# cloneofsimo/lora

Hardware: AMD Instinct MI355X
Metric: train steps/sec SD1.5 rank-4 512^2 (train_lora_dreambooth.py step) (higher is better)
Workload: dtype bf16

## Files before the change

include/lora_amd.h:

```cpp
#ifndef LORA_AMD_H
#define LORA_AMD_H

#include <stddef.h>
#include <stdint.h>

#ifdef __cplusplus
extern "C" {
#endif

#define LORA_AMD_ABI_VERSION 7

#define LORA_AMD_OK 0
#define LORA_AMD_EINVAL (-1)
#define LORA_AMD_ERANK (-2)
#define LORA_AMD_ELAUNCH (-3)
#define LORA_AMD_EWORKSPACE (-4)
#define LORA_AMD_EUNSUPPORTED (-5)

#define LORA_AMD_MAX_RANK 64

#define LORA_AMD_F32 0
#define LORA_AMD_F16 1
#define LORA_AMD_BF16 2

// ... 445 lines not shown
                                  int32_t r, int32_t act_dtype, float scale, float dropout_p, uint64_t seed, uint64_t offset,
                                  const uint64_t *offset_dev, void *stream);
int lora_amd_sum_parts(const float *part, int32_t nparts, int64_t stride, float *out, int64_t n, void *stream);


size_t lora_amd_sumsq_workspace(int64_t n);
int lora_amd_sumsq(const float *g, int64_t n, float *out_sumsq, void *workspace,
                   size_t workspace_bytes, void *stream);

typedef struct lora_amd_adamw_group {
  int64_t begin, end;
  float lr;
  float weight_decay;
} lora_amd_adamw_group;

int lora_amd_clip_adamw(float *p, float *g, float *exp_avg, float *exp_avg_sq,
                        int64_t n, const lora_amd_adamw_group *groups_dev,
                        int32_t n_groups, const float *sumsq, float grad_scale,
                        float max_norm, float beta1, float beta2, float eps,
                        int64_t step, int32_t zero_grad, void *stream);

int lora_amd_clip_adamw_dev(float *p, float *g, float *exp_avg, float *exp_avg_sq,
                            int64_t n, const lora_amd_adamw_group *groups_dev,
                            int32_t n_groups, const float *sumsq, float grad_scale,
                            float max_norm, float beta1, float beta2, float eps,
                            const int64_t *step_dev, const float *scaler, int32_t zero_grad, void *stream);
int lora_amd_step_advance(int64_t *step_dev, void *stream);

int lora_amd_loss_scale_update(float *state, const float *sumsq, int64_t *step_dev, float growth_factor,
                               float backoff_factor, int32_t growth_interval, void *stream);

int lora_amd_ti_rows_step(void *table, const void *table_grad, const int64_t *ids_dev, int32_t n_tokens,
                          int32_t hidden, int32_t table_dtype, float *rows, float *exp_avg, float *exp_avg_sq,
                          float lr, float beta1, float beta2, float eps, float weight_decay, float grad_scale,
                          int64_t step, float decay_lambda, float target_norm, void *stream);


size_t lora_amd_groupnorm_workspace(int32_t B, int32_t C, int32_t HW, int32_t groups);
int lora_amd_groupnorm_supported(int32_t B, int32_t C, int32_t HW, int32_t groups);
int lora_amd_groupnorm_fwd(const void *x, const void *gamma, const void *beta, void *y, float *stats,
                           void *workspace, size_t workspace_bytes, int32_t B, int32_t C, int32_t HW,
                           int32_t groups, float eps, int32_t act, int32_t dtype, void *stream);
int lora_amd_groupnorm_bwd(const void *x, const void *gout, const void *gamma, const void *beta,
                           const float *stats, void *dx, void *workspace, size_t workspace_bytes, int32_t B,
                           int32_t C, int32_t HW, int32_t groups, int32_t act, int32_t dtype, void *stream);

size_t lora_amd_groupnorm_nhwc_workspace(int32_t B, int32_t C, int32_t HW, int32_t groups);
int lora_amd_groupnorm_nhwc_fwd(const void *x, const void *gamma, const void *beta, const float *addend, void *y,
                                float *aff, void *workspace, size_t workspace_bytes, int32_t B, int32_t C, int32_t HW,
                                int32_t groups, float eps, int32_t act, int32_t dtype, void *stream);
int lora_amd_groupnorm_nhwc_bwd(const void *x, const void *gout, const void *gamma, const float *aff, void *dx,
                                void *workspace, size_t workspace_bytes, int32_t B, int32_t C, int32_t HW,
                                int32_t groups, int32_t act, int32_t dtype, void *stream);

int lora_amd_layernorm_supported(int32_t K);
int lora_amd_layernorm_fwd(const void *x, const void *gamma, const void *beta, void *y, float *stats, int64_t M,
                           int32_t K, float eps, int32_t dtype, void *stream);
int lora_amd_layernorm_bwd(const void *x, const void *gout, const void *gamma, const float *stats, void *dx,
                           int64_t M, int32_t K, int32_t dtype, void *stream);
int lora_amd_add_layernorm_fwd(const void *x, const void *res, const void *gamma, const void *beta, void *sum_out,
                               void *y, float *stats, int64_t M, int32_t K, float eps, int32_t dtype, void *stream);
int lora_amd_add_layernorm_bwd(const void *x, const void *gout, const void *gsum, const void *gamma,
                               const float *stats, void *dx, int64_t M, int32_t K, int32_t dtype, void *stream);

int lora_amd_geglu_fwd(const void *y, int64_t ldy, void *out, int64_t ldo, int64_t M, int32_t inner, int32_t dtype,
                       void *stream);
int lora_amd_geglu_bwd(const void *y, int64_t ldy, const void *gout, int64_t ldg, void *gy, int64_t ldgy, int64_t M,
                       int32_t inner, int32_t dtype, void *stream);

#ifdef __cplusplus
}
#endif
#endif
```

lora_amd/_C.py:

```python
from __future__ import annotations

import ctypes as C
import os
from typing import Dict, Optional, Sequence, Tuple

import torch

_HERE = os.path.dirname(os.path.abspath(__file__))
LIB_PATH = os.path.join(_HERE, "csrc", "liblora_amd.so")

OK = 0
F32, F16, BF16 = 0, 1, 2
FACTOR_RK, FACTOR_KR = 0, 1
ROUND_REFERENCE, ROUND_ONCE, ROUND_DITHER = 0, 1, 2
MAX_RANK = 64
ABI_VERSION = 7

_DT = {torch.float32: F32, torch.float16: F16, torch.bfloat16: BF16}

SYMBOLS = (
    "lora_amd_abi_version", "lora_amd_last_error", "lora_amd_target_arch",
    "lora_amd_merge_plan", "lora_amd_merge_batched", "lora_amd_merge_set_tuning", "lora_amd_merge_step_set_tuning", "lora_amd_rank16_mfma", "lora_amd_factors_mfma_set_tuning",
    "lora_amd_merge_step_plan", "lora_amd_merge_step",
    "lora_amd_rowdot", "lora_amd_rowdot_masked", "lora_amd_rank_update",
    "lora_amd_colreduce_workspace", "lora_amd_colreduce",
    "lora_amd_rowdot_batched", "lora_amd_colreduce_batched", "lora_amd_chol_inverse_batched",
    "lora_amd_ragged_plan", "lora_amd_rowdot_ragged", "lora_amd_colreduce_ragged", "lora_amd_sub_ragged",
    "lora_amd_rowdot16_planes_plan", "lora_amd_rowdot16_planes", "lora_amd_rowdot16_planes_packed", "lora_amd_thin_pack",
    "lora_amd_split16_ragged", "lora_amd_split16_transpose",
    "lora_amd_split16_residual", "lora_amd_thin_gram", "lora_amd_thin_apply", "lora_amd_thin_rotate", "lora_amd_thin_select", "lora_amd_thin_clamp",
    "lora_amd_linear_plan", "lora_amd_linear_fwd", "lora_amd_linear_bwd_g", "lora_amd_linear_bwd_x",
    "lora_amd_linear_bwd_factors", "lora_amd_linear_bwd_factors_drop", "lora_amd_linear_bwd_factors_heads",
    "lora_amd_linear_factors_self_plan", "lora_amd_linear_factors_self_plan_rows", "lora_amd_linear_bwd_factors_self",
    "lora_amd_linear_factors_self_ragged_plan", "lora_amd_linear_bwd_factors_self_ragged",
    "lora_amd_factors_mfma_plan", "lora_amd_factor_pack_plan", "lora_amd_factor_pack",
    "lora_amd_factors_mfma_ragged_plan", "lora_amd_linear_bwd_factors_mfma_ragged", "lora_amd_factors_mfma_block_map",
    "lora_amd_linear_bwd_factors_mfma_ragged_mapped",
    "lora_amd_linear_gemm_fwd_heads",
    "lora_amd_reduce_batched", "lora_amd_linear_gemm_supported", "lora_amd_linear_gemm_fwd",
    "lora_amd_ws_config", "lora_amd_ws_packed_elems", "lora_amd_ws_pack", "lora_amd_linear_ws", "lora_amd_linear_ws_heads",
    "lora_amd_conv_plan", "lora_amd_conv_down_fwd", "lora_amd_conv_up_fwd", "lora_amd_conv_bwd_g", "lora_amd_conv_bwd_x",
    "lora_amd_conv3_nhwc_plan", "lora_amd_conv3_nhwc_pack", "lora_amd_conv3_nhwc_down_fwd", "lora_amd_conv3_nhwc_bwd_dx",
    "lora_amd_conv3_nhwc_bwd_down", "lora_amd_sum_parts",
    "lora_amd_conv3_nhwc_pack_plan", "lora_amd_conv3_nhwc_pack_batched", "lora_amd_conv3_nhwc_fwd_fused",
    "lora_amd_linear_bwd_g_blocks", "lora_amd_linear_bwd_g_folded",
    "lora_amd_sumsq_workspace", "lora_amd_sumsq", "lora_amd_clip_adamw", "lora_amd_clip_adamw_dev",
    "lora_amd_step_advance", "lora_amd_loss_scale_update", "lora_amd_ti_rows_step",
    "lora_amd_groupnorm_workspace", "lora_amd_groupnorm_supported", "lora_amd_groupnorm_fwd", "lora_amd_groupnorm_bwd",
    "lora_amd_geglu_fwd", "lora_amd_geglu_bwd",
    "lora_amd_layernorm_supported", "lora_amd_layernorm_fwd", "lora_amd_layernorm_bwd",
    "lora_amd_groupnorm_nhwc_workspace", "lora_amd_groupnorm_nhwc_fwd", "lora_amd_groupnorm_nhwc_bwd",
    "lora_amd_add_layernorm_fwd", "lora_amd_add_layernorm_bwd",
    "lora_amd_linear_gemm_fwd_rowscale", "lora_amd_rank_update_rowscale", "lora_amd_conv_up_fwd_rowscale",
)


class HipExtensionMissing(RuntimeError):
    pass


class FactorsSelfPlan(C.Structure):
    _fields_ = [("supported", C.c_int32), ("rank_tile", C.c_int32), ("nparts", C.c_int32), ("reserved", C.c_int32),
                ("up_part_floats", C.c_int64), ("down_part_floats", C.c_int64)]


class SelfSite(C.Structure):
    _fields_ = [
        ("g", C.c_void_p), ("x", C.c_void_p), ("down", C.c_void_p), ("up", C.c_void_p),
        ("up_part", C.c_void_p), ("down_part", C.c_void_p),
        ("ldg", C.c_int64), ("ldx", C.c_int64), ("M", C.c_int64),
        ("N", C.c_int32), ("K", C.c_int32), ("r", C.c_int32), ("scale", C.c_float),
        ("g_head_dim", C.c_int32), ("g_head_pad", C.c_int32), ("x_head_dim", C.c_int32), ("x_head_pad", C.c_int32),
        ("rows_per_block", C.c_int32), ("nsplit", C.c_int32), ("kt_g", C.c_int32), ("logL_g", C.c_int32),
        ("kt_x", C.c_int32), ("logL_x", C.c_int32), ("tile_g", C.c_int32), ("nct_g", C.c_int32),
        ("tile_x", C.c_int32), ("nct_x", C.c_int32),
        ("reserved0", C.c_int32), ("reserved", C.c_int32),
        ("block_begin", C.c_int64),
    ]


class FactorsMfmaPlan(C.Structure):
    _fields_ = [("supported", C.c_int32), ("lds_class", C.c_int32), ("rank_tile", C.c_int32),
                ("rows_per_block", C.c_int32), ("nparts", C.c_int32), ("lds_bytes", C.c_int32),
                ("blocks_per_wg", C.c_int32), ("reserved", C.c_int32),
                ("up_part_floats", C.c_int64), ("down_part_floats", C.c_int64),
                ("pack_up_elems", C.c_int64), ("pack_down_elems", C.c_int64)]


class PackSite(C.Structure):
    _fields_ = [("down", C.c_void_p), ("up", C.c_void_p), ("pk_down", C.c_void_p), ("pk_up", C.c_void_p),
                ("N", C.c_int32), ("K", C.c_int32), ("r", C.c_int32), ("reserved", C.c_int32), ("begin", C.c_int64)]


class FmSite(C.Structure):
    _fields_ = [
        ("g", C.c_void_p), ("x", C.c_void_p), ("pk_up", C.c_void_p), ("pk_down", C.c_void_p),
        ("up_part", C.c_void_p), ("down_part", C.c_void_p),
        ("ldg", C.c_int64), ("ldx", C.c_int64), ("M", C.c_int64),
        ("N", C.c_int32), ("K", C.c_int32), ("r", C.c_int32), ("scale", C.c_float),
        ("g_head_dim", C.c_int32), ("g_head_pad", C.c_int32), ("x_head_dim", C.c_int32), ("x_head_pad", C.c_int32),
        ("rows_per_block", C.c_int32), ("blocks_per_wg", C.c_int32),
        ("resident_is_x", C.c_int32), ("cw", C.c_int32), ("nchunk", C.c_int32), ("x_head_magic", C.c_int32),
        ("g_head_magic", C.c_int32), ("lds_bytes", C.c_int32),
        ("block_begin", C.c_int64),
# ... 236 lines not shown
    lib.lora_amd_linear_gemm_supported.restype = lib.lora_amd_linear_gemm_fwd.restype = C.c_int
    lib.lora_amd_linear_gemm_fwd_rowscale.argtypes = [vp, i64, vp, i64, vp, vp, i64, vp, vp, vp, i64, i32, i32, i32, i32,
                                                      f32, vp, i32, i64, i32, vp]
    lib.lora_amd_rank_update_rowscale.argtypes = [vp, i64, vp, vp, i64, i32, i32, i32, i32, i32, f32, vp, i32, i64, f32,
                                                  u64, u64, vp]
    lib.lora_amd_conv_up_fwd_rowscale.argtypes = [vp, vp, vp, i32, i32, i32, i32, i32, i32, i32, f32, vp, i32, i64, f32,
                                                  u64, u64, vp]
    for name in ("lora_amd_linear_gemm_fwd_rowscale", "lora_amd_rank_update_rowscale", "lora_amd_conv_up_fwd_rowscale"):
        getattr(lib, name).restype = C.c_int
    lib.lora_amd_ws_config.argtypes = [i32, C.POINTER(i32), C.POINTER(i32)]
    lib.lora_amd_ws_packed_elems.argtypes = [i32, i32]
    lib.lora_amd_ws_packed_elems.restype = i64
    lib.lora_amd_ws_pack.argtypes = [vp, i64, i64, i32, i32, i32, vp, vp]
    lib.lora_amd_linear_ws.argtypes = [vp, i64, i64, i32, i32, C.POINTER(WsSite), i32, i32, vp]
    lib.lora_amd_linear_ws_heads.argtypes = [vp, i64, i64, i32, i32, i32, i32, C.POINTER(WsSite), i32, i32, vp]
    lib.lora_amd_ws_config.restype = lib.lora_amd_ws_pack.restype = lib.lora_amd_linear_ws.restype = C.c_int
    lib.lora_amd_linear_ws_heads.restype = C.c_int
    lib.lora_amd_conv_plan.argtypes = [i32, i32, i32, i32, i32, i32, i32, C.POINTER(ConvPlan)]
    lib.lora_amd_conv_down_fwd.argtypes = [vp, vp, vp, vp, vp, i32, i32, i32, i32, i32, i32, i32, i32, vp]
    lib.lora_amd_conv_up_fwd.argtypes = [vp, vp, vp, i32, i32, i32, i32, i32, i32, i32, f32, f32, u64, u64, vp, vp]
    lib.lora_amd_conv_bwd_g.argtypes = [vp, vp, vp, vp, vp, vp, vp, i32, i32, i32, i32, i32, i32, i32, f32, f32, u64,
                                        u64, vp, vp]
    lib.lora_amd_conv_bwd_x.argtypes = [vp, vp, vp, vp, vp, i32, i32, i32, i32, i32, i32, i32, i32, vp]
    lib.lora_amd_conv3_nhwc_plan.argtypes = [i32, i32, i32, i32, i32, C.POINTER(Conv3NhwcPlan)]
    lib.lora_amd_conv3_nhwc_pack.argtypes = [vp, i32, i32, i32, vp, vp, vp]
    lib.lora_amd_conv3_nhwc_down_fwd.argtypes = [vp, vp, vp, vp, i32, i32, i32, i32, i32, i32, vp]
    lib.lora_amd_conv3_nhwc_bwd_dx.argtypes = [vp, vp, vp, i32, i32, i32, i32, i32, i32, vp]
    lib.lora_amd_conv3_nhwc_bwd_down.argtypes = [vp, vp, vp, i32, i32, i32, i32, i32, i32, vp]
    lib.lora_amd_sum_parts.argtypes = [vp, i32, i64, vp, i64, vp]
    lib.lora_amd_conv3_nhwc_pack_plan.argtypes = [C.POINTER(Conv3PackSite), i32, C.POINTER(i64)]
    lib.lora_amd_conv3_nhwc_pack_batched.argtypes = [vp, i32, i64, i32, vp]
    lib.lora_amd_conv3_nhwc_fwd_fused.argtypes = [vp, vp, vp, vp, vp, vp, vp, i32, i32, i32, i32, i32, i32, i32, f32, f32,
                                                  u64, u64, vp, vp]
    lib.lora_amd_linear_bwd_g_blocks.argtypes = [i64, i32, i32, C.POINTER(i64)]
    lib.lora_amd_linear_bwd_g_folded.argtypes = [vp, i64, vp, vp, vp, vp, vp, vp, i64, i32, i32, i32, i32, f32, f32, u64,
                                                 u64, vp, vp]
    for name in ("lora_amd_conv3_nhwc_plan", "lora_amd_conv3_nhwc_pack", "lora_amd_conv3_nhwc_down_fwd",
                 "lora_amd_conv3_nhwc_bwd_dx", "lora_amd_conv3_nhwc_bwd_down", "lora_amd_sum_parts",
                 "lora_amd_conv3_nhwc_pack_plan", "lora_amd_conv3_nhwc_pack_batched", "lora_amd_conv3_nhwc_fwd_fused",
                 "lora_amd_linear_bwd_g_blocks", "lora_amd_linear_bwd_g_folded"):
        getattr(lib, name).restype = C.c_int
    lib.lora_amd_groupnorm_workspace.argtypes = [i32, i32, i32, i32]
    lib.lora_amd_groupnorm_workspace.restype = sz
    lib.lora_amd_groupnorm_supported.argtypes = [i32, i32, i32, i32]
    lib.lora_amd_groupnorm_fwd.argtypes = [vp, vp, vp, vp, vp, vp, sz, i32, i32, i32, i32, f32, i32, i32, vp]
    lib.lora_amd_groupnorm_bwd.argtypes = [vp, vp, vp, vp, vp, vp, vp, sz, i32, i32, i32, i32, i32, i32, vp]
    lib.lora_amd_geglu_fwd.argtypes = [vp, i64, vp, i64, i64, i32, i32, vp]
    lib.lora_amd_geglu_bwd.argtypes = [vp, i64, vp, i64, vp, i64, i64, i32, i32, vp]
    lib.lora_amd_groupnorm_nhwc_workspace.argtypes = [i32, i32, i32, i32]
    lib.lora_amd_groupnorm_nhwc_workspace.restype = sz
    lib.lora_amd_groupnorm_nhwc_fwd.argtypes = [vp, vp, vp, vp, vp, vp, vp, sz, i32, i32, i32, i32, f32, i32, i32, vp]
    lib.lora_amd_groupnorm_nhwc_bwd.argtypes = [vp, vp, vp, vp, vp, vp, sz, i32, i32, i32, i32, i32, i32, vp]
    lib.lora_amd_groupnorm_nhwc_fwd.restype = lib.lora_amd_groupnorm_nhwc_bwd.restype = C.c_int
    lib.lora_amd_add_layernorm_fwd.argtypes = [vp, vp, vp, vp, vp, vp, vp, i64, i32, f32, i32, vp]
    lib.lora_amd_add_layernorm_bwd.argtypes = [vp, vp, vp, vp, vp, vp, i64, i32, i32, vp]
    lib.lora_amd_add_layernorm_fwd.restype = lib.lora_amd_add_layernorm_bwd.restype = C.c_int
    lib.lora_amd_layernorm_supported.argtypes = [i32]
    lib.lora_amd_layernorm_fwd.argtypes = [vp, vp, vp, vp, vp, i64, i32, f32, i32, vp]
    lib.lora_amd_layernorm_bwd.argtypes = [vp, vp, vp, vp, vp, i64, i32, i32, vp]
    for name in ("lora_amd_groupnorm_supported", "lora_amd_groupnorm_fwd", "lora_amd_groupnorm_bwd",
                 "lora_amd_geglu_fwd", "lora_amd_geglu_bwd", "lora_amd_layernorm_supported",
                 "lora_amd_layernorm_fwd", "lora_amd_layernorm_bwd"):
        getattr(lib, name).restype = C.c_int
    for name in ("lora_amd_conv_plan", "lora_amd_conv_down_fwd", "lora_amd_conv_up_fwd", "lora_amd_conv_bwd_g",
                 "lora_amd_conv_bwd_x"):
        getattr(lib, name).restype = C.c_int
    for name in ("lora_amd_linear_plan", "lora_amd_linear_fwd", "lora_amd_linear_bwd_g", "lora_amd_linear_bwd_x",
                 "lora_amd_reduce_batched"):
        getattr(lib, name).restype = C.c_int
    for name in ("lora_amd_merge_plan", "lora_amd_merge_batched", "lora_amd_merge_set_tuning", "lora_amd_rowdot",
                 "lora_amd_rowdot_masked", "lora_amd_rank_update", "lora_amd_colreduce", "lora_amd_sumsq",
                 "lora_amd_clip_adamw"):
        getattr(lib, name).restype = C.c_int


def load() -> Optional[C.CDLL]:
    global _lib, _load_error
    if _lib is not None or _load_error is not None:
        return _lib
    if not os.path.exists(LIB_PATH):
        _load_error = f"{LIB_PATH} not built (run `python -c 'import __graft_entry__ as g; g.build()'`)"
        return None
    try:
        lib = C.CDLL(LIB_PATH)
        _declare(lib)
        if lib.lora_amd_abi_version() != ABI_VERSION:
            raise OSError(f"ABI version {lib.lora_amd_abi_version()} != {ABI_VERSION} (rebuild: make -C lora_amd/csrc)")
        _lib = lib
    except OSError as e:
        _load_error = f"cannot load {LIB_PATH}: {e}"
    return _lib


def available() -> bool:
    return load() is not None


def require() -> C.CDLL:
    lib = load()
    if lib is None:
        raise HipExtensionMissing(
            "lora_amd: the HIP extension is required for device tensors and is not loadable: " + str(_load_error))
    return lib


def _check(rc: int, what: str) -> None:
# ... 1534 lines not shown
    gy = torch.empty(y.shape, dtype=y.dtype, device=y.device)
    _check(require().lora_amd_geglu_bwd(y2.data_ptr(), y2.stride(0), g2.data_ptr(), g2.stride(0), gy.data_ptr(),
                                        2 * inner, y2.shape[0], inner, dtype_code(y.dtype), _stream()),
           "lora_amd_geglu_bwd")
    return gy


def layernorm_supported(K: int) -> bool:
    return bool(require().lora_amd_layernorm_supported(K))


def layernorm_fwd(x: torch.Tensor, gamma: torch.Tensor, beta: torch.Tensor, eps: float, *,
                  out: Optional[torch.Tensor] = None, stats: Optional[torch.Tensor] = None) -> Tuple[torch.Tensor, torch.Tensor]:
    _dev_check(x, gamma, beta, out, stats)
    K = x.shape[-1]
    M = x.numel() // K
    if out is None:
        y = torch.empty_like(x)
    elif out.dtype != x.dtype or out.shape != x.shape or not out.is_contiguous():
        raise ValueError("layernorm_fwd: out must be a contiguous tensor of x's shape and dtype")
    else:
        y = out
    if stats is None:
        stats = torch.empty(M, 2, dtype=torch.float32, device=x.device)
    elif stats.dtype != torch.float32 or tuple(stats.shape) != (M, 2) or not stats.is_contiguous():
        raise ValueError(f"layernorm_fwd: stats must be a contiguous f32 [{M}, 2] tensor")
    _check(require().lora_amd_layernorm_fwd(x.data_ptr(), gamma.data_ptr(), beta.data_ptr(), y.data_ptr(),
                                            stats.data_ptr(), M, K, eps, dtype_code(x.dtype), _stream()),
           "lora_amd_layernorm_fwd")
    return y, stats


def layernorm_bwd(x: torch.Tensor, gout: torch.Tensor, gamma: torch.Tensor, stats: torch.Tensor) -> torch.Tensor:
    _dev_check(x, gout, gamma, stats)
    K = x.shape[-1]
    dx = torch.empty_like(x)
    _check(require().lora_amd_layernorm_bwd(x.data_ptr(), gout.data_ptr(), gamma.data_ptr(), stats.data_ptr(),
                                            dx.data_ptr(), x.numel() // K, K, dtype_code(x.dtype), _stream()),
           "lora_amd_layernorm_bwd")
    return dx


_gn_nhwc_ws_cache: Dict[Tuple[int, int, int, int], int] = {}


def groupnorm_nhwc_workspace(B: int, C_: int, HW: int, groups: int) -> int:
    key = (B, C_, HW, groups)
    n = _gn_nhwc_ws_cache.get(key)
    if n is None:
        n = _gn_nhwc_ws_cache[key] = int(require().lora_amd_groupnorm_nhwc_workspace(B, C_, HW, groups))
    return n


def groupnorm_nhwc_fwd(x: torch.Tensor, gamma: torch.Tensor, beta: torch.Tensor, groups: int, eps: float,
                       act: bool, addend: Optional[torch.Tensor] = None) -> Tuple[torch.Tensor, torch.Tensor]:
    _dev_check(x, gamma, beta, addend)
    if addend is not None and (addend.dtype != torch.float32 or not addend.is_contiguous()
                               or tuple(addend.shape) != (x.shape[0], x.shape[1])):
        raise ValueError("groupnorm_nhwc_fwd: addend must be a contiguous float32 [B, C] tensor")
    B, C_ = x.shape[0], x.shape[1]
    HW = x.numel() // (B * C_)
    nbytes = groupnorm_nhwc_workspace(B, C_, HW, groups)
    if nbytes == 0:
        raise ValueError(f"lora_amd_groupnorm_nhwc: geometry {tuple(x.shape)} / {groups} groups not supported")
    y = torch.empty_like(x)
    aff = torch.empty(B, 4, C_, dtype=torch.float32, device=x.device)
    ws = torch.empty(nbytes // 4, dtype=torch.float32, device=x.device)
    _check(require().lora_amd_groupnorm_nhwc_fwd(x.data_ptr(), gamma.data_ptr(), beta.data_ptr(), _ptr(addend),
                                                 y.data_ptr(), aff.data_ptr(), ws.data_ptr(), nbytes, B, C_, HW, groups, eps,
                                                 1 if act else 0, dtype_code(x.dtype), _stream()),
           "lora_amd_groupnorm_nhwc_fwd")
    return y, aff


def groupnorm_nhwc_bwd(x: torch.Tensor, gout: torch.Tensor, gamma: torch.Tensor, aff: torch.Tensor, groups: int,
                       act: bool) -> torch.Tensor:
    _dev_check(x, gout, gamma, aff)
    B, C_ = x.shape[0], x.shape[1]
    HW = x.numel() // (B * C_)
    nbytes = groupnorm_nhwc_workspace(B, C_, HW, groups)
    dx = torch.empty_like(x)
    ws = torch.empty(nbytes // 4, dtype=torch.float32, device=x.device)
    _check(require().lora_amd_groupnorm_nhwc_bwd(x.data_ptr(), gout.data_ptr(), gamma.data_ptr(), aff.data_ptr(),
                                                 dx.data_ptr(), ws.data_ptr(), nbytes, B, C_, HW, groups,
                                                 1 if act else 0, dtype_code(x.dtype), _stream()),
           "lora_amd_groupnorm_nhwc_bwd")
    return dx


def add_layernorm_fwd(x: torch.Tensor, res: torch.Tensor, gamma: torch.Tensor, beta: torch.Tensor,
                      eps: float) -> Tuple[torch.Tensor, torch.Tensor, torch.Tensor]:
    _dev_check(x, res, gamma, beta)
    K = x.shape[-1]
    M = x.numel() // K
    s, y = torch.empty_like(x), torch.empty_like(x)
    stats = torch.empty(M, 2, dtype=torch.float32, device=x.device)
    _check(require().lora_amd_add_layernorm_fwd(x.data_ptr(), res.data_ptr(), gamma.data_ptr(), beta.data_ptr(),
                                                s.data_ptr(), y.data_ptr(), stats.data_ptr(), M, K, eps,
                                                dtype_code(x.dtype), _stream()), "lora_amd_add_layernorm_fwd")
    return s, y, stats


def add_layernorm_bwd(s: torch.Tensor, gout: torch.Tensor, gsum: Optional[torch.Tensor], gamma: torch.Tensor,
                      stats: torch.Tensor) -> torch.Tensor:
    _dev_check(s, gout, gsum, gamma, stats)
    K = s.shape[-1]
    dx = torch.empty_like(s)
    _check(require().lora_amd_add_layernorm_bwd(s.data_ptr(), gout.data_ptr(), _ptr(gsum), gamma.data_ptr(),
                                                stats.data_ptr(), dx.data_ptr(), s.numel() // K, K,
                                                dtype_code(s.dtype), _stream()), "lora_amd_add_layernorm_bwd")
    return dx
```

lora_amd/csrc/hostops.hip:

```cpp
#include <algorithm>

#include "common.hpp"

namespace lora_amd {

constexpr int kHT = 256;
constexpr int kHU = 4;
constexpr int kHMaxSlices = 256;

__device__ inline float fast_rcp(float v) { return __builtin_amdgcn_rcpf(v); }
__device__ inline float sigmoidf(float z) { return fast_rcp(1.f + __expf(-z)); }
__device__ inline float silu_grad(float z) {
  const float s = sigmoidf(z);
  return s * (1.f + z * (1.f - s));
}
__device__ inline float erf_as(float x) {
  const float ax = fabsf(x);
  const float t = fast_rcp(1.f + 0.3275911f * ax);
  float p = 1.061405429f;
  p = fmaf(p, t, -1.453152027f);
  p = fmaf(p, t, 1.421413741f);
  p = fmaf(p, t, -0.284496736f);
  p = fmaf(p, t, 0.254829592f);
  const float e = 1.f - p * t * __expf(-ax * ax);
// ... 752 lines not shown
      }
      LORA_AMD_LOADS_ISSUED();
#pragma unroll
      for (int u = 0; u < kNU; ++u) {
        const int pp = p + u * nslots;
        if (pp < k.np) {
          float v[8], go[8], t[8], xh[8];
          unpack8_sel<E>(xr[u], true, v);
          unpack8_sel<E>(gr[u], true, go);
          gn_nhwc_terms<E, ACT>(v, go, ga, be, mean, rstd, gam, t, xh);
          if (APPLY) {
            float o[8];
#pragma unroll
            for (int e = 0; e < 8; ++e) o[e] = rstd[e] * (t[e] - c1[e] - xh[e] * c2[e]);
            store8<E>(dx + k.base + (int64_t)pp * C, o);
          } else {
#pragma unroll
            for (int e = 0; e < 8; ++e) {
              s1[e] += t[e];
              s2[e] = fmaf(t[e], xh[e], s2[e]);
            }
          }
        }
      }
    }
  }
  if (!APPLY) {
    nhwc_slot_reduce(s1, s2, k, cw, nslots, s_red);
    if (k.active && k.slot == 0) {
      float *o = part + ((int64_t)(k.b * S + k.s) * 2) * C + (int64_t)k.col * 8;
      st8f(o, s1);
      st8f(o + C, s2);
    }
  }
}

__global__ __launch_bounds__(kHT) void gn_nhwc_bwd_finalize_kernel(const float *__restrict__ part,
                                                                   float *__restrict__ cvec, int C, int HW, int G,
                                                                   int S) {
  __shared__ float s_red[4][2];
  const int b = blockIdx.x / G, g = blockIdx.x - b * G, cpg = C / G;
  float s1 = 0.f, s2 = 0.f;
  for (int i = threadIdx.x; i < S * cpg; i += kHT) {
    const int s = i / cpg, c = g * cpg + (i - s * cpg);
    const float *pp = part + ((int64_t)(b * S + s) * 2) * C + c;
    s1 += pp[0];
    s2 += pp[C];
  }
  block_sum2(s1, s2, s_red);
  const float inv_n = 1.f / ((float)HW * (float)cpg);
  for (int cc = threadIdx.x; cc < cpg; cc += kHT) {
    cvec[(int64_t)b * 2 * C + g * cpg + cc] = s1 * inv_n;
    cvec[(int64_t)b * 2 * C + C + g * cpg + cc] = s2 * inv_n;
  }
}

static inline bool aligned_for(const void *p, int dt) { return ((uintptr_t)p % (dt == LORA_AMD_F32 ? 32 : 16)) == 0; }

}

using namespace lora_amd;

extern "C" size_t lora_amd_groupnorm_workspace(int32_t B, int32_t C, int32_t HW, int32_t groups) {
  const GnGeo q = gn_geo(B, C, HW, groups);
  return q.ok ? (size_t)B * groups * q.S * 2 * sizeof(float) : 0;
}

extern "C" int lora_amd_groupnorm_supported(int32_t B, int32_t C, int32_t HW, int32_t groups) {
  return gn_geo(B, C, HW, groups).ok ? 1 : 0;
}

#define GN_CHECKS(name)                                                                                              \
  const GnGeo q = gn_geo(B, C, HW, groups);                                                                          \
  LORA_AMD_CHECK(q.ok, LORA_AMD_EINVAL, name ": geometry B=%d C=%d HW=%d groups=%d not supported", B, C, HW, groups); \
  LORA_AMD_CHECK(dtype_ok(dtype), LORA_AMD_EINVAL, name ": bad dtype %d", dtype);                                    \
  LORA_AMD_CHECK(workspace_bytes >= lora_amd_groupnorm_workspace(B, C, HW, groups), LORA_AMD_EWORKSPACE,             \
                 name ": workspace %zu < %zu bytes", workspace_bytes, lora_amd_groupnorm_workspace(B, C, HW, groups)); \
  const dim3 grid((unsigned)((int64_t)B * groups * q.S)), block(kHT);                                                \
  hipStream_t st = (hipStream_t)stream;                                                                              \
  float *part = reinterpret_cast<float *>(workspace)

extern "C" int lora_amd_groupnorm_fwd(const void *x, const void *gamma, const void *beta, void *y, float *stats,
                                      void *workspace, size_t workspace_bytes, int32_t B, int32_t C, int32_t HW,
                                      int32_t groups, float eps, int32_t act, int32_t dtype, void *stream) {
  GN_CHECKS("groupnorm_fwd");
  LORA_AMD_CHECK(x && gamma && beta && y && stats && workspace, LORA_AMD_EINVAL, "groupnorm_fwd: null pointer");
  LORA_AMD_CHECK(aligned_for(x, dtype) && aligned_for(y, dtype), LORA_AMD_EINVAL, "groupnorm_fwd: unaligned tensor");
  by_dtype(dtype, [&](auto e) {
    using E = decltype(e);
    using S = typename E::storage;
    hipLaunchKernelGGL((gn_stats_kernel<E>), grid, block, 0, st, (const S *)x, part, groups, q.cpg, HW, q.chunks,
                       q.per_block, q.S);
    by_bool(act != 0, [&](auto a) {
      hipLaunchKernelGGL((gn_apply_kernel<E, decltype(a)::value>), grid, block, 0, st, (const S *)x, (const S *)gamma,
                         (const S *)beta, (S *)y, part, stats, groups, q.cpg, HW, q.chunks, q.per_block, q.S, eps);
    });
  });
  return check_launch("lora_amd_groupnorm_fwd");
}

extern "C" int lora_amd_groupnorm_bwd(const void *x, const void *gout, const void *gamma, const void *beta,
                                      const float *stats, void *dx, void *workspace, size_t workspace_bytes,
                                      int32_t B, int32_t C, int32_t HW, int32_t groups, int32_t act, int32_t dtype,
                                      void *stream) {
  GN_CHECKS("groupnorm_bwd");
  LORA_AMD_CHECK(x && gout && gamma && beta && stats && dx && workspace, LORA_AMD_EINVAL,
// ... 77 lines not shown
}

extern "C" int lora_amd_add_layernorm_fwd(const void *x, const void *res, const void *gamma, const void *beta,
                                          void *sum_out, void *y, float *stats, int64_t M, int32_t K, float eps,
                                          int32_t dtype, void *stream) {
  LN_CHECKS("layernorm_fwd");
  LORA_AMD_CHECK(x && gamma && beta && y && stats, LORA_AMD_EINVAL, "layernorm_fwd: null pointer");
  LORA_AMD_CHECK((res == nullptr) == (sum_out == nullptr), LORA_AMD_EINVAL,
                 "layernorm_fwd: res and sum_out go together");
  LORA_AMD_CHECK(aligned_for(x, dtype) && aligned_for(y, dtype) && aligned_for(gamma, dtype) && aligned_for(beta, dtype) &&
                     aligned_for(res, dtype) && aligned_for(sum_out, dtype),
                 LORA_AMD_EINVAL, "layernorm_fwd: unaligned tensor");
  const bool add = res != nullptr;
  by_dtype(dtype, [&](auto e) {
    by_bool(add, [&](auto a) {
      using S = typename decltype(e)::storage;
      hipLaunchKernelGGL((ln_fwd_kernel<decltype(e), decltype(a)::value>), grid, block, 0, st, (const S *)x, (const S *)res,
                         (const S *)gamma, (const S *)beta, (S *)sum_out, (S *)y, stats, M, c8, logL, eps);
    });
  });
  return check_launch("lora_amd_layernorm_fwd");
}

extern "C" int lora_amd_layernorm_bwd(const void *x, const void *gout, const void *gamma, const float *stats,
                                      void *dx, int64_t M, int32_t K, int32_t dtype, void *stream) {
  return lora_amd_add_layernorm_bwd(x, gout, nullptr, gamma, stats, dx, M, K, dtype, stream);
}

extern "C" int lora_amd_add_layernorm_bwd(const void *x, const void *gout, const void *gsum, const void *gamma,
                                          const float *stats, void *dx, int64_t M, int32_t K, int32_t dtype,
                                          void *stream) {
  LN_CHECKS("layernorm_bwd");
  LORA_AMD_CHECK(x && gout && gamma && stats && dx, LORA_AMD_EINVAL, "layernorm_bwd: null pointer");
  LORA_AMD_CHECK(aligned_for(x, dtype) && aligned_for(gout, dtype) && aligned_for(dx, dtype) && aligned_for(gamma, dtype) &&
                     aligned_for(gsum, dtype),
                 LORA_AMD_EINVAL, "layernorm_bwd: unaligned tensor");
  by_dtype(dtype, [&](auto e) {
    by_bool(gsum != nullptr, [&](auto a) {
      using S = typename decltype(e)::storage;
      hipLaunchKernelGGL((ln_bwd_kernel<decltype(e), decltype(a)::value>), grid, block, 0, st, (const S *)x, (const S *)gout,
                         (const S *)gsum, (const S *)gamma, stats, (S *)dx, M, c8, logL);
    });
  });
  return check_launch("lora_amd_layernorm_bwd");
}

static size_t gn_nhwc_part_floats(const GnNhwcGeo &q, int B, int C) { return (size_t)B * q.S * 2 * C; }

extern "C" size_t lora_amd_groupnorm_nhwc_workspace(int32_t B, int32_t C, int32_t HW, int32_t groups) {
  const GnNhwcGeo q = gn_nhwc_geo(B, C, HW, groups);
  return q.ok ? (gn_nhwc_part_floats(q, B, C) + (size_t)B * 2 * C) * sizeof(float) : 0;
}

#define GN_NHWC_CHECKS(name)                                                                                          \
  const GnNhwcGeo q = gn_nhwc_geo(B, C, HW, groups);                                                                  \
  LORA_AMD_CHECK(q.ok, LORA_AMD_EINVAL, name ": geometry B=%d C=%d HW=%d groups=%d not supported", B, C, HW, groups); \
  LORA_AMD_CHECK(dtype_ok(dtype), LORA_AMD_EINVAL, name ": bad dtype %d", dtype);                                     \
  LORA_AMD_CHECK(workspace_bytes >= lora_amd_groupnorm_nhwc_workspace(B, C, HW, groups), LORA_AMD_EWORKSPACE,         \
                 name ": workspace %zu bytes too small", workspace_bytes);                                            \
  const dim3 grid((unsigned)((int64_t)B * q.S * q.tiles)), gridg((unsigned)(B * groups)), block(kHT);                 \
  hipStream_t st = (hipStream_t)stream;                                                                               \
  float *part = reinterpret_cast<float *>(workspace);                                                                 \
  float *cvec = part + gn_nhwc_part_floats(q, B, C);                                                                  \
  (void)cvec

extern "C" int lora_amd_groupnorm_nhwc_fwd(const void *x, const void *gamma, const void *beta, const float *addend,
                                           void *y, float *aff, void *workspace, size_t workspace_bytes, int32_t B, int32_t C, int32_t HW,
                                           int32_t groups, float eps, int32_t act, int32_t dtype, void *stream) {
  GN_NHWC_CHECKS("groupnorm_nhwc_fwd");
  LORA_AMD_CHECK(x && gamma && beta && y && aff && workspace, LORA_AMD_EINVAL, "groupnorm_nhwc_fwd: null pointer");
  LORA_AMD_CHECK(aligned_for(x, dtype) && aligned_for(y, dtype) && ((uintptr_t)aff % 32) == 0, LORA_AMD_EINVAL,
                 "groupnorm_nhwc_fwd: unaligned tensor");
  by_dtype(dtype, [&](auto e) {
    using E = decltype(e);
    using S = typename E::storage;
    hipLaunchKernelGGL((gn_nhwc_stats_kernel<E>), grid, block, 0, st, (const S *)x, part, C, HW, q.cw, q.tiles,
                       q.nslots, q.px, q.S);
    hipLaunchKernelGGL((gn_nhwc_finalize_kernel<E>), gridg, block, 0, st, part, (const S *)gamma, (const S *)beta,
                       addend, aff, C, HW, groups, q.px, q.S, eps);
    by_bool(act != 0, [&](auto a) {
      hipLaunchKernelGGL((gn_nhwc_apply_kernel<E, decltype(a)::value>), grid, block, 0, st, (const S *)x, aff, (S *)y, C, HW,
                         q.cw, q.tiles, q.nslots, q.px, q.S);
    });
  });
  return check_launch("lora_amd_groupnorm_nhwc_fwd");
}

extern "C" int lora_amd_groupnorm_nhwc_bwd(const void *x, const void *gout, const void *gamma, const float *aff,
                                           void *dx, void *workspace, size_t workspace_bytes, int32_t B, int32_t C,
                                           int32_t HW, int32_t groups, int32_t act, int32_t dtype, void *stream) {
  GN_NHWC_CHECKS("groupnorm_nhwc_bwd");
  LORA_AMD_CHECK(x && gout && gamma && aff && dx && workspace, LORA_AMD_EINVAL, "groupnorm_nhwc_bwd: null pointer");
  LORA_AMD_CHECK(aligned_for(x, dtype) && aligned_for(gout, dtype) && aligned_for(dx, dtype) &&
                     aligned_for(gamma, dtype) && ((uintptr_t)aff % 32) == 0,
                 LORA_AMD_EINVAL, "groupnorm_nhwc_bwd: unaligned tensor");
  by_dtype(dtype, [&](auto e) {
    by_bool(act != 0, [&](auto a) {
      using E = decltype(e);
      using S = typename E::storage;
      constexpr bool A = decltype(a)::value;
      hipLaunchKernelGGL((gn_nhwc_bwd_kernel<E, A, false>), grid, block, 0, st, (const S *)x, (const S *)gout,
                         (const S *)gamma, aff, part, (const float *)nullptr, (S *)nullptr, C, HW, q.cw, q.tiles,
                         q.nslots, q.px, q.S);
      hipLaunchKernelGGL(gn_nhwc_bwd_finalize_kernel, gridg, block, 0, st, part, cvec, C, HW, groups, q.S);
      hipLaunchKernelGGL((gn_nhwc_bwd_kernel<E, A, true>), grid, block, 0, st, (const S *)x, (const S *)gout,
                         (const S *)gamma, aff, (float *)nullptr, cvec, (S *)dx, C, HW, q.cw, q.tiles, q.nslots,
                         q.px, q.S);
    });
  });
  return check_launch("lora_amd_groupnorm_nhwc_bwd");
}
```

Before: 35.30.

## Add single-kernel register-resident NHWC GroupNorm path for small slabs

Adds a resident GroupNorm forward and backward kernel in which one block holds a whole group slab in registers. It computes the mean, variance and apply (or the backward reductions and dx) in a single launch, replacing the three-kernel stats/finalize/apply pipeline. It also skips the workspace allocation when the resident path is chosen. A router with an auto mode enables the path only when the slab is at most 40KB, and a host-side cache remembers the choice per shape. The trade-off is higher register pressure and lower parallelism per group on larger shapes, which the size threshold is meant to avoid.

```diff
diff --git a/include/lora_amd.h b/include/lora_amd.h
--- a/include/lora_amd.h
+++ b/include/lora_amd.h
@@ -521,6 +521,8 @@
 int lora_amd_groupnorm_nhwc_bwd(const void *x, const void *gout, const void *gamma, const float *aff, void *dx,
                                 void *workspace, size_t workspace_bytes, int32_t B, int32_t C, int32_t HW,
                                 int32_t groups, int32_t act, int32_t dtype, void *stream);
+int lora_amd_groupnorm_nhwc_route(int32_t B, int32_t C, int32_t HW, int32_t groups, int32_t dtype, int32_t backward);
+int lora_amd_groupnorm_nhwc_set_route(int32_t mode);
 
 int lora_amd_layernorm_supported(int32_t K);
 int lora_amd_layernorm_fwd(const void *x, const void *gamma, const void *beta, void *y, float *stats, int64_t M,
diff --git a/lora_amd/_C.py b/lora_amd/_C.py
--- a/lora_amd/_C.py
+++ b/lora_amd/_C.py
@@ -50,6 +50,7 @@
     "lora_amd_geglu_fwd", "lora_amd_geglu_bwd",
     "lora_amd_layernorm_supported", "lora_amd_layernorm_fwd", "lora_amd_layernorm_bwd",
     "lora_amd_groupnorm_nhwc_workspace", "lora_amd_groupnorm_nhwc_fwd", "lora_amd_groupnorm_nhwc_bwd",
+    "lora_amd_groupnorm_nhwc_route", "lora_amd_groupnorm_nhwc_set_route",
     "lora_amd_add_layernorm_fwd", "lora_amd_add_layernorm_bwd",
     "lora_amd_linear_gemm_fwd_rowscale", "lora_amd_rank_update_rowscale", "lora_amd_conv_up_fwd_rowscale",
 )
@@ -392,6 +393,9 @@
     lib.lora_amd_groupnorm_nhwc_fwd.argtypes = [vp, vp, vp, vp, vp, vp, vp, sz, i32, i32, i32, i32, f32, i32, i32, vp]
     lib.lora_amd_groupnorm_nhwc_bwd.argtypes = [vp, vp, vp, vp, vp, vp, sz, i32, i32, i32, i32, i32, i32, vp]
     lib.lora_amd_groupnorm_nhwc_fwd.restype = lib.lora_amd_groupnorm_nhwc_bwd.restype = C.c_int
+    lib.lora_amd_groupnorm_nhwc_route.argtypes = [i32, i32, i32, i32, i32, i32]
+    lib.lora_amd_groupnorm_nhwc_set_route.argtypes = [i32]
+    lib.lora_amd_groupnorm_nhwc_route.restype = lib.lora_amd_groupnorm_nhwc_set_route.restype = C.c_int
     lib.lora_amd_add_layernorm_fwd.argtypes = [vp, vp, vp, vp, vp, vp, vp, i64, i32, f32, i32, vp]
     lib.lora_amd_add_layernorm_bwd.argtypes = [vp, vp, vp, vp, vp, vp, i64, i32, i32, vp]
     lib.lora_amd_add_layernorm_fwd.restype = lib.lora_amd_add_layernorm_bwd.restype = C.c_int
@@ -2032,6 +2036,30 @@
     return n
 
 
+_gn_nhwc_route_cache: Dict[Tuple[int, int, int, int, int, bool], int] = {}
+
+
+def groupnorm_nhwc_route(B: int, C_: int, HW: int, groups: int, dtype: torch.dtype, backward: bool) -> int:
+    key = (B, C_, HW, groups, dtype_code(dtype), bool(backward))
+    r = _gn_nhwc_route_cache.get(key)
+    if r is None:
+        r = _gn_nhwc_route_cache[key] = int(require().lora_amd_groupnorm_nhwc_route(B, C_, HW, groups, key[4],
+                                                                                     1 if backward else 0))
+    return r
+
+
+def groupnorm_nhwc_set_route(mode: int) -> int:
+    _gn_nhwc_route_cache.clear()
+    return int(require().lora_amd_groupnorm_nhwc_set_route(int(mode)))
+
+
+def _gn_nhwc_ws(B: int, C_: int, HW: int, groups: int, x: torch.Tensor, backward: bool):
+    if groupnorm_nhwc_route(B, C_, HW, groups, x.dtype, backward) == 1:
+        return None, 0
+    nbytes = groupnorm_nhwc_workspace(B, C_, HW, groups)
+    return torch.empty(nbytes // 4, dtype=torch.float32, device=x.device), nbytes
+
+
 def groupnorm_nhwc_fwd(x: torch.Tensor, gamma: torch.Tensor, beta: torch.Tensor, groups: int, eps: float,
                        act: bool, addend: Optional[torch.Tensor] = None) -> Tuple[torch.Tensor, torch.Tensor]:
     _dev_check(x, gamma, beta, addend)
@@ -2040,14 +2068,13 @@
         raise ValueError("groupnorm_nhwc_fwd: addend must be a contiguous float32 [B, C] tensor")
     B, C_ = x.shape[0], x.shape[1]
     HW = x.numel() // (B * C_)
-    nbytes = groupnorm_nhwc_workspace(B, C_, HW, groups)
-    if nbytes == 0:
+    if groupnorm_nhwc_workspace(B, C_, HW, groups) == 0:
         raise ValueError(f"lora_amd_groupnorm_nhwc: geometry {tuple(x.shape)} / {groups} groups not supported")
     y = torch.empty_like(x)
     aff = torch.empty(B, 4, C_, dtype=torch.float32, device=x.device)
-    ws = torch.empty(nbytes // 4, dtype=torch.float32, device=x.device)
+    ws, nbytes = _gn_nhwc_ws(B, C_, HW, groups, x, False)
     _check(require().lora_amd_groupnorm_nhwc_fwd(x.data_ptr(), gamma.data_ptr(), beta.data_ptr(), _ptr(addend),
-                                                 y.data_ptr(), aff.data_ptr(), ws.data_ptr(), nbytes, B, C_, HW, groups, eps,
+                                                 y.data_ptr(), aff.data_ptr(), _ptr(ws), nbytes, B, C_, HW, groups, eps,
                                                  1 if act else 0, dtype_code(x.dtype), _stream()),
            "lora_amd_groupnorm_nhwc_fwd")
     return y, aff
@@ -2058,11 +2085,10 @@
     _dev_check(x, gout, gamma, aff)
     B, C_ = x.shape[0], x.shape[1]
     HW = x.numel() // (B * C_)
-    nbytes = groupnorm_nhwc_workspace(B, C_, HW, groups)
     dx = torch.empty_like(x)
-    ws = torch.empty(nbytes // 4, dtype=torch.float32, device=x.device)
+    ws, nbytes = _gn_nhwc_ws(B, C_, HW, groups, x, True)
     _check(require().lora_amd_groupnorm_nhwc_bwd(x.data_ptr(), gout.data_ptr(), gamma.data_ptr(), aff.data_ptr(),
-                                                 dx.data_ptr(), ws.data_ptr(), nbytes, B, C_, HW, groups,
+                                                 dx.data_ptr(), _ptr(ws), nbytes, B, C_, HW, groups,
                                                  1 if act else 0, dtype_code(x.dtype), _stream()),
            "lora_amd_groupnorm_nhwc_bwd")
     return dx
diff --git a/lora_amd/csrc/hostops.hip b/lora_amd/csrc/hostops.hip
--- a/lora_amd/csrc/hostops.hip
+++ b/lora_amd/csrc/hostops.hip
@@ -828,6 +828,309 @@
   for (int cc = threadIdx.x; cc < cpg; cc += kHT) {
     cvec[(int64_t)b * 2 * C + g * cpg + cc] = s1 * inv_n;
     cvec[(int64_t)b * 2 * C + C + g * cpg + cc] = s2 * inv_n;
+  }
+}
+
+constexpr int kGnResFwdT = 1024;
+constexpr int kGnResBwdT = 512;
+constexpr int gn_res_max_pieces(bool f32, bool backward) { return f32 ? 4 : backward ? 6 : 8; }
+
+struct GnResGeo {
+  int cpg, R, cw, np, nslots, threads;
+  uint64_t inv_cw, inv_cpg;
+  bool ok;
+};
+static GnResGeo gn_res_geo(int B, int C, int HW, int G, int dtype, bool backward) {
+  GnResGeo r{};
+  if (!gn_nhwc_geo(B, C, HW, G).ok || !dtype_ok(dtype)) return r;
+  r.cpg = C / G;
+  int gcd8 = 8;
+  while (r.cpg % gcd8) gcd8 >>= 1;
+  r.R = 8 / gcd8;
+  r.cw = r.R * r.cpg / 8;
+  const int max_t = backward ? kGnResBwdT : kGnResFwdT;
+  const int max_np = gn_res_max_pieces(dtype == LORA_AMD_F32, backward);
+  for (int np : {1, 2, 4, 6, 8}) {
+    if (np > max_np) break;
+    const int64_t nslots = ((int64_t)HW + np - 1) / np;
+    if (nslots * r.cw > max_t) continue;
+    r.np = np;
+    r.nslots = (int)nslots;
+    r.threads = (r.nslots * r.cw + 63) / 64 * 64;
+    r.inv_cw = (1ull << 32) / (uint64_t)r.cw + 1;
+    r.inv_cpg = (1ull << 32) / (uint64_t)r.cpg + 1;
+    r.ok = true;
+    return r;
+  }
+  return r;
+}
+
+__device__ inline int gn_res_div(int n, uint64_t inv) { return (int)(((uint64_t)(unsigned)n * inv) >> 32); }
+
+struct GnResThread {
+  int b, slot, cl, c0;
+  int g_lo, nb;
+  bool active;
+  int64_t base;
+};
+__device__ inline GnResThread gn_res_thread(int C, int HW, int cpg, int cw, int nslots, uint64_t inv_cw, uint64_t inv_cpg) {
+  GnResThread k;
+  const int runs = C / (cw * 8);
+  k.b = blockIdx.x / runs;
+  const int run = blockIdx.x - k.b * runs;
+  k.slot = gn_res_div(threadIdx.x, inv_cw);
+  k.cl = threadIdx.x - k.slot * cw;
+  k.active = k.slot < nslots;
+  k.c0 = (run * cw + k.cl) * 8;
+  k.base = (int64_t)k.b * HW * C + k.c0;
+  k.g_lo = gn_res_div(k.cl * 8, inv_cpg);
+  k.nb = (k.g_lo + 1) * cpg - k.cl * 8;
+  return k;
+}
+__device__ inline void gn_res_fold(const float (&v)[8], const GnResThread &k, int cpg, uint64_t inv_cpg, float (&g)[8]) {
+  if (cpg >= 8) {
+    float lo = 0.f, hi = 0.f;
+#pragma unroll
+    for (int e = 0; e < 8; ++e) {
+      lo += e < k.nb ? v[e] : 0.f;
+      hi += e < k.nb ? 0.f : v[e];
+    }
+#pragma unroll
+    for (int r = 0; r < 8; ++r) g[r] = (k.g_lo == r ? lo : 0.f) + (k.g_lo + 1 == r ? hi : 0.f);
+  } else {
+#pragma unroll
+    for (int r = 0; r < 8; ++r) g[r] = 0.f;
+#pragma unroll
+    for (int e = 0; e < 8; ++e) {
+      const int gi = gn_res_div(k.cl * 8 + e, inv_cpg);
+#pragma unroll
+      for (int r = 0; r < 8; ++r) g[r] += gi == r ? v[e] : 0.f;
+    }
+  }
+}
+__device__ inline void gn_res_expand(const float (&g)[8], const GnResThread &k, int cpg, uint64_t inv_cpg, float (&v)[8]) {
+  if (cpg >= 8) {
+    float lo = g[0], hi = g[1];
+#pragma unroll
+    for (int r = 1; r < 8; ++r) lo = k.g_lo == r ? g[r] : lo;
+#pragma unroll
+    for (int r = 2; r < 8; ++r) hi = k.g_lo + 1 == r ? g[r] : hi;
+#pragma unroll
+    for (int e = 0; e < 8; ++e) v[e] = e < k.nb ? lo : hi;
+  } else {
+#pragma unroll
+    for (int e = 0; e < 8; ++e) {
+      const int gi = gn_res_div(k.cl * 8 + e, inv_cpg);
+      v[e] = g[0];
+#pragma unroll
+      for (int r = 1; r < 8; ++r) v[e] = gi == r ? g[r] : v[e];
+    }
+  }
+}
+template <class E, int NP>
+__device__ inline void gn_res_keep_packed(Raw8<E> (&raw)[NP]) {
+#pragma unroll
+  for (int j = 0; j < NP; ++j) asm volatile("" : "+v"(raw[j].v));
+}
+template <bool TWO>
+__device__ inline void gn_res_block_sum(float (&a)[8], float (&b)[8], int R, float (*s_a)[8], float (*s_b)[8]) {
+  const int wave = threadIdx.x >> 6, lane = threadIdx.x & 63, nwaves = blockDim.x >> 6;
+#pragma unroll
+  for (int r = 0; r < 8; ++r) {
+    if (r < R) {
+#pragma unroll
+      for (int off = 32; off > 0; off >>= 1) {
+        a[r] += __shfl_xor(a[r], off, 64);
+        if (TWO) b[r] += __shfl_xor(b[r], off, 64);
+      }
+      if (lane == 0) {
+        s_a[wave][r] = a[r];
+        if (TWO) s_b[wave][r] = b[r];
+      }
+    }
+  }
+  __syncthreads();
+  const int w = lane & 15;
+#pragma unroll
+  for (int r = 0; r < 8; ++r) {
+    if (r < R) {
+      a[r] = w < nwaves ? s_a[w][r] : 0.f;
+      if (TWO) b[r] = w < nwaves ? s_b[w][r] : 0.f;
+#pragma unroll
+      for (int off = 8; off > 0; off >>= 1) {
+        a[r] += __shfl_xor(a[r], off, 64);
+        if (TWO) b[r] += __shfl_xor(b[r], off, 64);
+      }
+    }
+  }
+}
+template <class E>
+__device__ inline void gn_res_load_vec(const typename E::storage *__restrict__ p, float (&v)[8]) {
+  if (((uintptr_t)p % (sizeof(typename E::storage) * 8)) == 0) {
+    unpack8_sel<E>(load8_raw<E>(p), true, v);
+  } else {
+#pragma unroll
+    for (int e = 0; e < 8; ++e) v[e] = E::to_f(p[e]);
+  }
+}
+
+template <class E, bool ACT, int NP>
+__global__ __launch_bounds__(kGnResFwdT) void gn_nhwc_resident_fwd_kernel(
+    const typename E::storage *__restrict__ x, const typename E::storage *__restrict__ gamma,
+    const typename E::storage *__restrict__ beta, const float *__restrict__ addend, typename E::storage *__restrict__ y,
+    float *__restrict__ aff, int C, int HW, int cpg, int R, int cw, int nslots, uint64_t inv_cw, uint64_t inv_cpg,
+    float eps) {
+  __shared__ float s_sum[16][8], s_m2[16][8];
+  const GnResThread k = gn_res_thread(C, HW, cpg, cw, nslots, inv_cw, inv_cpg);
+  Raw8<E> raw[NP];
+#pragma unroll
+  for (int j = 0; j < NP; ++j) {
+    const int p = k.slot + j * nslots;
+    raw[j] = load8_raw<E>(x + k.base + (int64_t)(k.active && p < HW ? p : 0) * C);
+  }
+  float gam[8], bet[8], add[8];
+  gn_res_load_vec<E>(gamma + k.c0, gam);
+  gn_res_load_vec<E>(beta + k.c0, bet);
+  if (addend != nullptr) {
+    gn_res_load_vec<f32_t>(addend + (int64_t)k.b * C + k.c0, add);
+  } else {
+#pragma unroll
+    for (int e = 0; e < 8; ++e) add[e] = 0.f;
+  }
+  LORA_AMD_LOADS_ISSUED();
+  float acc[8], g[8], unused[8], mean[8], rstd[8];
+#pragma unroll
+  for (int e = 0; e < 8; ++e) acc[e] = 0.f;
+#pragma unroll
+  for (int j = 0; j < NP; ++j) {
+    const bool ok = k.active && k.slot + j * nslots < HW;
+    float v[8];
+    unpack8_sel<E>(raw[j], true, v);
+#pragma unroll
+    for (int e = 0; e < 8; ++e) acc[e] += ok ? v[e] + add[e] : 0.f;
+  }
+  gn_res_fold(acc, k, cpg, inv_cpg, g);
+  gn_res_block_sum<false>(g, unused, R, s_sum, s_sum);
+  const float inv_n = 1.f / ((float)HW * (float)cpg);
+#pragma unroll
+  for (int r = 0; r < 8; ++r) g[r] *= inv_n;
+  gn_res_expand(g, k, cpg, inv_cpg, mean);
+  gn_res_keep_packed<E, NP>(raw);
+#pragma unroll
+  for (int e = 0; e < 8; ++e) acc[e] = 0.f;
+#pragma unroll
+  for (int j = 0; j < NP; ++j) {
+    const bool ok = k.active && k.slot + j * nslots < HW;
+    float v[8];
+    unpack8_sel<E>(raw[j], true, v);
+#pragma unroll
+    for (int e = 0; e < 8; ++e) {
+      const float d = (v[e] + add[e]) - mean[e];
+      acc[e] = ok ? fmaf(d, d, acc[e]) : acc[e];
+    }
+  }
+  gn_res_fold(acc, k, cpg, inv_cpg, g);
+  gn_res_block_sum<false>(g, unused, R, s_m2, s_m2);
+#pragma unroll
+  for (int r = 0; r < 8; ++r) g[r] = rsqrtf(g[r] * inv_n + eps);
+  gn_res_expand(g, k, cpg, inv_cpg, rstd);
+  gn_res_keep_packed<E, NP>(raw);
+  float ga[8], be[8];
+#pragma unroll
+  for (int e = 0; e < 8; ++e) {
+    ga[e] = gam[e] * rstd[e];
+    be[e] = fmaf(add[e] - mean[e], ga[e], bet[e]);
+    mean[e] -= add[e];
+  }
+  if (k.active && k.slot == 0) {
+    float *o = aff + (int64_t)k.b * 4 * C + k.c0;
+    st8f(o, ga);
+    st8f(o + C, be);
+    st8f(o + 2 * C, mean);
+    st8f(o + 3 * C, rstd);
+  }
+#pragma unroll
+  for (int j = 0; j < NP; ++j) {
+    const int p = k.slot + j * nslots;
+    if (k.active && p < HW) {
+      float v[8], o[8];
+      unpack8_sel<E>(raw[j], true, v);
+#pragma unroll
+      for (int e = 0; e < 8; ++e) {
+        const float z = fmaf(v[e], ga[e], be[e]);
+        o[e] = ACT ? z * sigmoidf(z) : z;
+      }
+      store8<E>(y + k.base + (int64_t)p * C, o);
+    }
+  }
+}
+
+template <class E, bool ACT, int NP>
+__global__ __launch_bounds__(kGnResBwdT) void gn_nhwc_resident_bwd_kernel(
+    const typename E::storage *__restrict__ x, const typename E::storage *__restrict__ gout,
+    const typename E::storage *__restrict__ gamma, const float *__restrict__ aff, typename E::storage *__restrict__ dx,
+    int C, int HW, int cpg, int R, int cw, int nslots, uint64_t inv_cw, uint64_t inv_cpg) {
+  __shared__ float s_1[16][8], s_2[16][8];
+  const GnResThread k = gn_res_thread(C, HW, cpg, cw, nslots, inv_cw, inv_cpg);
+  Raw8<E> xr[NP], gr[NP];
+#pragma unroll
+  for (int j = 0; j < NP; ++j) {
+    const int p = k.slot + j * nslots;
+    const int64_t off = k.base + (int64_t)(k.active && p < HW ? p : 0) * C;
+    xr[j] = load8_raw<E>(x + off);
+    gr[j] = load8_raw<E>(gout + off);
+  }
+  float ga[8], be[8], mean[8], rstd[8], gam[8], s1[8], s2[8], c1[8], c2[8];
+  const float *ab = aff + (int64_t)k.b * 4 * C + k.c0;
+  ld8f(ab, ga);
+  ld8f(ab + C, be);
+  ld8f(ab + 2 * C, mean);
+  ld8f(ab + 3 * C, rstd);
+  unpack8_sel<E>(load8_raw<E>(gamma + k.c0), true, gam);
+  LORA_AMD_LOADS_ISSUED();
+#pragma unroll
+  for (int e = 0; e < 8; ++e) s1[e] = s2[e] = 0.f;
+#pragma unroll
+  for (int j = 0; j < NP; ++j) {
+    const bool ok = k.active && k.slot + j * nslots < HW;
+    float v[8], go[8], t[8], xh[8];
+    unpack8_sel<E>(xr[j], true, v);
+    unpack8_sel<E>(gr[j], true, go);
+    gn_nhwc_terms<E, ACT>(v, go, ga, be, mean, rstd, gam, t, xh);
+#pragma unroll
+    for (int e = 0; e < 8; ++e) {
+      s1[e] += ok ? t[e] : 0.f;
+      s2[e] = ok ? fmaf(t[e], xh[e], s2[e]) : s2[e];
+    }
+    __builtin_amdgcn_sched_barrier(0);
+  }
+  float g1[8], g2[8];
+  gn_res_fold(s1, k, cpg, inv_cpg, g1);
+  gn_res_fold(s2, k, cpg, inv_cpg, g2);
+  gn_res_block_sum<true>(g1, g2, R, s_1, s_2);
+  const float inv_n = 1.f / ((float)HW * (float)cpg);
+#pragma unroll
+  for (int r = 0; r < 8; ++r) {
+    g1[r] *= inv_n;
+    g2[r] *= inv_n;
+  }
+  gn_res_expand(g1, k, cpg, inv_cpg, c1);
+  gn_res_expand(g2, k, cpg, inv_cpg, c2);
+  gn_res_keep_packed<E, NP>(xr);
+  gn_res_keep_packed<E, NP>(gr);
+#pragma unroll
+  for (int j = 0; j < NP; ++j) {
+    const int p = k.slot + j * nslots;
+    if (k.active && p < HW) {
+      float v[8], go[8], t[8], xh[8], o[8];
+      unpack8_sel<E>(xr[j], true, v);
+      unpack8_sel<E>(gr[j], true, go);
+      gn_nhwc_terms<E, ACT>(v, go, ga, be, mean, rstd, gam, t, xh);
+#pragma unroll
+      for (int e = 0; e < 8; ++e) o[e] = rstd[e] * (t[e] - c1[e] - xh[e] * c2[e]);
+      store8<E>(dx + k.base + (int64_t)p * C, o);
+    }
+    __builtin_amdgcn_sched_barrier(0);
   }
 }
 
@@ -1011,28 +1314,70 @@
   return q.ok ? (gn_nhwc_part_floats(q, B, C) + (size_t)B * 2 * C) * sizeof(float) : 0;
 }
 
-#define GN_NHWC_CHECKS(name)                                                                                          \
+static int g_gn_route = 0;
+constexpr int64_t kGnResAutoSlabBytes = 40 * 1024;
+
+static GnResGeo gn_res_route(int B, int C, int HW, int G, int dtype, bool backward) {
+  GnResGeo r = gn_res_geo(B, C, HW, G, dtype, backward);
+  if (g_gn_route == 1) r.ok = false;
+  if (g_gn_route == 0 && r.ok)
+    r.ok = (int64_t)HW * r.cw * 8 * (dtype == LORA_AMD_F32 ? 4 : 2) <= kGnResAutoSlabBytes;
+  return r;
+}
+
+extern "C" int lora_amd_groupnorm_nhwc_route(int32_t B, int32_t C, int32_t HW, int32_t groups, int32_t dtype,
+                                             int32_t backward) {
+  return gn_res_route(B, C, HW, groups, dtype, backward != 0).ok ? 1 : 0;
+}
+
+extern "C" int lora_amd_groupnorm_nhwc_set_route(int32_t mode) {
+  const int prev = g_gn_route;
+  if (mode >= 0 && mode <= 2) g_gn_route = mode;
+  return prev;
+}
+
+#define GN_NHWC_CHECKS(name, backward)                                                                                \
   const GnNhwcGeo q = gn_nhwc_geo(B, C, HW, groups);                                                                  \
   LORA_AMD_CHECK(q.ok, LORA_AMD_EINVAL, name ": geometry B=%d C=%d HW=%d groups=%d not supported", B, C, HW, groups); \
   LORA_AMD_CHECK(dtype_ok(dtype), LORA_AMD_EINVAL, name ": bad dtype %d", dtype);                                     \
-  LORA_AMD_CHECK(workspace_bytes >= lora_amd_groupnorm_nhwc_workspace(B, C, HW, groups), LORA_AMD_EWORKSPACE,         \
-                 name ": workspace %zu bytes too small", workspace_bytes);                                            \
+  const GnResGeo res = gn_res_route(B, C, HW, groups, dtype, backward);                                               \
+  LORA_AMD_CHECK(res.ok || workspace_bytes >= lora_amd_groupnorm_nhwc_workspace(B, C, HW, groups),                    \
+                 LORA_AMD_EWORKSPACE, name ": workspace %zu bytes too small", workspace_bytes);                       \
+  LORA_AMD_CHECK(res.ok || workspace, LORA_AMD_EINVAL, name ": null workspace");                                      \
   const dim3 grid((unsigned)((int64_t)B * q.S * q.tiles)), gridg((unsigned)(B * groups)), block(kHT);                 \
+  const dim3 grid_res((unsigned)(res.ok ? (int64_t)B * (groups / res.R) : 1)), block_res(res.ok ? res.threads : 64);  \
   hipStream_t st = (hipStream_t)stream;                                                                               \
   float *part = reinterpret_cast<float *>(workspace);                                                                 \
   float *cvec = part + gn_nhwc_part_floats(q, B, C);                                                                  \
   (void)cvec
 
+template <class E, bool BACKWARD, class F>
+static void gn_res_by_pieces(int np, F &&f) {
+  by_int<1, 2, 4, 6, 8>(np, [&](auto n) {
+    if constexpr (decltype(n)::value <= gn_res_max_pieces(sizeof(typename E::storage) == 4, BACKWARD)) f(n);
+  });
+}
+
 extern "C" int lora_amd_groupnorm_nhwc_fwd(const void *x, const void *gamma, const void *beta, const float *addend,
                                            void *y, float *aff, void *workspace, size_t workspace_bytes, int32_t B, int32_t C, int32_t HW,
                                            int32_t groups, float eps, int32_t act, int32_t dtype, void *stream) {
-  GN_NHWC_CHECKS("groupnorm_nhwc_fwd");
-  LORA_AMD_CHECK(x && gamma && beta && y && aff && workspace, LORA_AMD_EINVAL, "groupnorm_nhwc_fwd: null pointer");
+  GN_NHWC_CHECKS("groupnorm_nhwc_fwd", false);
+  LORA_AMD_CHECK(x && gamma && beta && y && aff, LORA_AMD_EINVAL, "groupnorm_nhwc_fwd: null pointer");
   LORA_AMD_CHECK(aligned_for(x, dtype) && aligned_for(y, dtype) && ((uintptr_t)aff % 32) == 0, LORA_AMD_EINVAL,
                  "groupnorm_nhwc_fwd: unaligned tensor");
   by_dtype(dtype, [&](auto e) {
     using E = decltype(e);
     using S = typename E::storage;
+    if (res.ok) {
+      by_bool(act != 0, [&](auto a) {
+        gn_res_by_pieces<E, false>(res.np, [&](auto n) {
+          hipLaunchKernelGGL((gn_nhwc_resident_fwd_kernel<E, decltype(a)::value, decltype(n)::value>), grid_res, block_res, 0,
+                             st, (const S *)x, (const S *)gamma, (const S *)beta, addend, (S *)y, aff, C, HW, res.cpg,
+                             res.R, res.cw, res.nslots, res.inv_cw, res.inv_cpg, eps);
+        });
+      });
+      return;
+    }
     hipLaunchKernelGGL((gn_nhwc_stats_kernel<E>), grid, block, 0, st, (const S *)x, part, C, HW, q.cw, q.tiles,
                        q.nslots, q.px, q.S);
     hipLaunchKernelGGL((gn_nhwc_finalize_kernel<E>), gridg, block, 0, st, part, (const S *)gamma, (const S *)beta,
@@ -1048,8 +1393,8 @@
 extern "C" int lora_amd_groupnorm_nhwc_bwd(const void *x, const void *gout, const void *gamma, const float *aff,
                                            void *dx, void *workspace, size_t workspace_bytes, int32_t B, int32_t C,
                                            int32_t HW, int32_t groups, int32_t act, int32_t dtype, void *stream) {
-  GN_NHWC_CHECKS("groupnorm_nhwc_bwd");
-  LORA_AMD_CHECK(x && gout && gamma && aff && dx && workspace, LORA_AMD_EINVAL, "groupnorm_nhwc_bwd: null pointer");
+  GN_NHWC_CHECKS("groupnorm_nhwc_bwd", true);
+  LORA_AMD_CHECK(x && gout && gamma && aff && dx, LORA_AMD_EINVAL, "groupnorm_nhwc_bwd: null pointer");
   LORA_AMD_CHECK(aligned_for(x, dtype) && aligned_for(gout, dtype) && aligned_for(dx, dtype) &&
                      aligned_for(gamma, dtype) && ((uintptr_t)aff % 32) == 0,
                  LORA_AMD_EINVAL, "groupnorm_nhwc_bwd: unaligned tensor");
@@ -1058,6 +1403,14 @@
       using E = decltype(e);
       using S = typename E::storage;
       constexpr bool A = decltype(a)::value;
+      if (res.ok) {
+        gn_res_by_pieces<E, true>(res.np, [&](auto n) {
+          hipLaunchKernelGGL((gn_nhwc_resident_bwd_kernel<E, A, decltype(n)::value>), grid_res, block_res, 0, st,
+                             (const S *)x, (const S *)gout, (const S *)gamma, aff, (S *)dx, C, HW, res.cpg, res.R, res.cw,
+                             res.nslots, res.inv_cw, res.inv_cpg);
+        });
+        return;
+      }
       hipLaunchKernelGGL((gn_nhwc_bwd_kernel<E, A, false>), grid, block, 0, st, (const S *)x, (const S *)gout,
                          (const S *)gamma, aff, part, (const float *)nullptr, (S *)nullptr, C, HW, q.cw, q.tiles,
                          q.nslots, q.px, q.S);
```

Result: no change. 35.64, median of 6 (+1.0%).
